# NBDsoftware/deep_cartograph

Measured on AMD Instinct MI355X. Metric: Deep-TICA training frames/sec on 10Mx512 feature matrix at 1/2/4/8 GPUs, higher is better.
Workload: dtype f32

## Files before the change

deep_cartograph_amd/csrc/gemm.h:

```cpp
#pragma once
#include <type_traits>
#include "common.h"
#include "handoff.h"

namespace dcv {

#ifdef DCV_STAMP
__device__ unsigned long long g_stamp[8 * 8192];
#define DCV_STAMP_AT(slot)                                                                      \
    do {                                                                                        \
        if (threadIdx.x == 0 && blockIdx.x < 8192 && blockIdx.z == 0)                           \
            g_stamp[blockIdx.x * 8 + (slot)] = __builtin_amdgcn_s_memtime();                   \
    } while (0)
#define DCV_STAMP_RT(slot)                                                                      \
    do {                                                                                        \
        if (threadIdx.x == 0 && blockIdx.x < 8192 && blockIdx.z == 0)                           \
            g_stamp[blockIdx.x * 8 + (slot)] = __builtin_amdgcn_s_memrealtime();               \
    } while (0)
#else
#define DCV_STAMP_AT(slot) do {} while (0)
#define DCV_STAMP_RT(slot) do {} while (0)
#endif

typedef float f32x16 __attribute__((ext_vector_type(16)));
typedef float v4f __attribute__((ext_vector_type(4)));
typedef unsigned u32x4 __attribute__((ext_vector_type(4)));
typedef __bf16 bf16x8 __attribute__((ext_vector_type(8)));

__device__ __forceinline__ void split3(const float (&x)[8], u32x4& p1, u32x4& p2, u32x4& p3) {
#pragma unroll
    for (int i = 0; i < 4; ++i) {
        const unsigned a = __float_as_uint(x[2 * i]), b = __float_as_uint(x[2 * i + 1]);
        p1[i] = __builtin_amdgcn_perm(b, a, 0x07060302);
        const float ra = x[2 * i] - __uint_as_float(a & 0xFFFF0000u);
        const float rb = x[2 * i + 1] - __uint_as_float(b & 0xFFFF0000u);
        const unsigned a2 = __float_as_uint(ra), b2 = __float_as_uint(rb);
        p2[i] = __builtin_amdgcn_perm(b2, a2, 0x07060302);
        const float sa = ra - __uint_as_float(a2 & 0xFFFF0000u);
        const float sb = rb - __uint_as_float(b2 & 0xFFFF0000u);
        p3[i] = __builtin_amdgcn_perm(__float_as_uint(sb), __float_as_uint(sa), 0x07060302);
    }
}
__device__ __forceinline__ bf16x8 as_bf16x8(const u32x4& v) { return __builtin_bit_cast(bf16x8, v); }

enum GemmMode { kNT = 0, kNN = 1, kTN = 2 };

template <class E, class = void> struct epi_has_asum : std::false_type {};
template <class E> struct epi_has_asum<E, std::void_t<decltype(E::kASum)>> : std::bool_constant<E::kASum> {};

struct RowMap {
    const int64_t* idx;
    int64_t row0;
    int32_t half;
    int32_t lag;
    template <bool GATHER>
    __device__ __forceinline__ int64_t get(int64_t r) const {
        const bool second = half > 0 && r >= half;
        const int64_t j = second ? r - half : r;
        int64_t base;
        if constexpr (GATHER) base = idx ? idx[j] : row0 + j;
        else base = row0 + j;
        return second ? base + lag : base;
    }
};
inline RowMap identity_rows() { return RowMap{nullptr, 0, 0, 0}; }

struct Operand {
    const float* p;
    int64_t ld;
    RowMap rows;
    const float* shift;
    int vec_ok;
    int planes = 0;
    int64_t pstride = 0;
};

struct GemmDims {
    int64_t M, N, K;
    int64_t k_chunk;
    int tiles_m, tiles_n;
    int xcd_remap;
    int wt;
    int tail_split = 0;
    float* tail_ws = nullptr;
    unsigned* tail_cnt = nullptr;
};

template <int WAVES_M_, int WAVES_N_, int FM_, int FN_, int KB_, int NBUF_ = 2, bool SPLIT_ = false, int PL_ = 0>
struct TileCfg {
    static constexpr int WAVES_M = WAVES_M_, WAVES_N = WAVES_N_, FM = FM_, FN = FN_, KB = KB_, NBUF = NBUF_;
    static constexpr bool SPLIT = SPLIT_;
    static constexpr int PL = PL_;
    static_assert(PL == 0 || SPLIT, "plane operands belong to the split flavour");
    static constexpr bool LS = (PL_ & 16) != 0;
    static constexpr int RAW_SZ = LS ? (WAVES_M_ * FM_ * 32 + WAVES_N_ * FN_ * 32) * KB_ : 0;
    static constexpr int A_SZ = (PL & 5) ? 3 * (WAVES_M_ * FM_ * 32) * (KB_ / 2) : (WAVES_M_ * FM_ * 32) * KB_;
    static constexpr int B_SZ = (PL & 10) ? 3 * (WAVES_N_ * FN_ * 32) * (KB_ / 2) : (WAVES_N_ * FN_ * 32) * KB_;
    static_assert(NBUF >= 2 && NBUF <= 8, "NBUF");
    static constexpr int TM = WAVES_M * FM * 32;
    static constexpr int TN = WAVES_N * FN * 32;
    static_assert(WAVES_M * WAVES_N == 4, "4 waves per workgroup");
    static_assert(KB == 16 || KB == 32, "KB");
};

template <int KB>
__device__ __forceinline__ int mmajor_off(int row, int chunk) {
    constexpr int CPR = KB / 4;
    constexpr int RPBR = 64 / KB;
    return row * KB + ((chunk ^ ((row / RPBR) % CPR)) << 2);
}

__device__ __forceinline__ void glds16(const float* gsrc, unsigned lds_wave_addr) {
    unsigned keep;
    asm volatile(
        "s_mov_b32 %0, m0\n\t"
        "s_mov_b32 m0, %2\n\t"
        "s_nop 0\n\t"
        "global_load_lds_dwordx4 %1, off\n\t"
        "s_mov_b32 m0, %0"
        : "=&s"(keep)
        : "v"(gsrc), "s"(lds_wave_addr)
        : "memory");
}
__device__ __forceinline__ unsigned lds_addr_uniform(const float* p) {
    const unsigned a = (unsigned)(uintptr_t)(__attribute__((address_space(3))) const float*)p;
    return __builtin_amdgcn_readfirstlane(a);
}

template <int PER>
__device__ __forceinline__ void glds16_batch(const float* base, const unsigned (&voff)[PER], unsigned lds0) {
    static_assert(PER == 1 || PER == 2 || PER == 4, "units per thread");
    unsigned keep;
    if constexpr (PER == 1) {
        asm volatile(
            "s_mov_b32 %0, m0\n\ts_nop 3\n\t"
            "s_mov_b32 m0, %3\n\ts_nop 0\n\tglobal_load_lds_dwordx4 %1, %2\n\t"
            "s_mov_b32 m0, %0"
            : "=&s"(keep)
            : "v"(voff[0]), "s"(base), "s"(lds0)
            : "memory");
    } else if constexpr (PER == 2) {
        asm volatile(
            "s_mov_b32 %0, m0\n\ts_nop 3\n\t"
            "s_mov_b32 m0, %4\n\ts_nop 0\n\tglobal_load_lds_dwordx4 %1, %3\n\t"
            "s_mov_b32 m0, %5\n\ts_nop 0\n\tglobal_load_lds_dwordx4 %2, %3\n\t"
            "s_mov_b32 m0, %0"
            : "=&s"(keep)
            : "v"(voff[0]), "v"(voff[1]), "s"(base), "s"(lds0), "s"(lds0 + 4096u)
            : "memory");
    } else {
        asm volatile(
            "s_mov_b32 %0, m0\n\ts_nop 3\n\t"
            "s_mov_b32 m0, %6\n\ts_nop 0\n\tglobal_load_lds_dwordx4 %1, %5\n\t"
            "s_mov_b32 m0, %7\n\ts_nop 0\n\tglobal_load_lds_dwordx4 %2, %5\n\t"
            "s_mov_b32 m0, %8\n\ts_nop 0\n\tglobal_load_lds_dwordx4 %3, %5\n\t"
            "s_mov_b32 m0, %9\n\ts_nop 0\n\tglobal_load_lds_dwordx4 %4, %5\n\t"
            "s_mov_b32 m0, %0"
            : "=&s"(keep)
            : "v"(voff[0]), "v"(voff[1]), "v"(voff[2]), "v"(voff[3]), "s"(base), "s"(lds0), "s"(lds0 + 4096u),
              "s"(lds0 + 8192u), "s"(lds0 + 12288u)
            : "memory");
    }
}
constexpr int64_t kMaxAffineLd = (int64_t)1 << 22;

template <int T, int KB, bool VEC, bool GATHER>
struct MMajorStage {
    static constexpr int CPR = KB / 4;
    static constexpr int RPBR = 64 / KB;
    static constexpr int UNITS = T * CPR;
    static constexpr int PER = (UNITS + 255) / 256;
    static_assert(256 % CPR == 0 && ((256 / CPR) / RPBR) % CPR == 0, "swizzle must not depend on the unit index");
    float4 r[PER];
    const float* src[PER];
    unsigned voff[PER];
// ... 431 lines not shown
    };
    float sha[FM], shb[FN];
    bool dma_sub = false;
#pragma unroll
    for (int i = 0; i < FM; ++i) sha[i] = 0.f;
#pragma unroll
    for (int j = 0; j < FN; ++j) shb[j] = 0.f;
    if constexpr (!A_MM) {
        if (A.shift) {
            dma_sub = true;
#pragma unroll
            for (int i = 0; i < FM; ++i) {
                const int64_t c = m0 + wm + i * 32 + (lane & 31);
                sha[i] = c < d.M ? A.shift[c] : 0.f;
            }
        }
    }
    if constexpr (!B_MM) {
        if (B.shift) {
            dma_sub = true;
#pragma unroll
            for (int j = 0; j < FN; ++j) {
                const int64_t c = n0 + wn + j * 32 + (lane & 31);
                shb[j] = c < d.N ? B.shift[c] : 0.f;
            }
        }
    }
    auto read_frags = [&](Frags& f, const float* la, const float* lb, int g) {
#pragma unroll
        for (int i = 0; i < FM; ++i) {
            if constexpr (A_MM) {
                f.a[i] = frag_mmajor<KB>(la, wm + i * 32, g, lane);
            } else {
#pragma unroll
                for (int s = 0; s < 4; ++s) f.a[i][s] = frag_kmajor<TM>(la, wm + i * 32, g, s, lane);
            }
        }
#pragma unroll
        for (int b = 0; b < NB; ++b)
#pragma unroll
            for (int j = 0; j < FN; ++j) {
                if constexpr (B_MM) {
                    f.b[b][j] = frag_mmajor<KB>(lb, wn + j * 32, g, lane);
                } else {
#pragma unroll
                    for (int s = 0; s < 4; ++s) f.b[b][j][s] = frag_kmajor<TN>(lb + b * B_SZ, wn + j * 32, g, s, lane);
                }
            }
    };
    auto sub_frags = [&](Frags& f) {
        if constexpr (!A_MM) {
#pragma unroll
            for (int i = 0; i < FM; ++i)
#pragma unroll
                for (int s = 0; s < 4; ++s) f.a[i][s] -= sha[i];
        }
        if constexpr (!B_MM) {
#pragma unroll
            for (int b = 0; b < NB; ++b)
#pragma unroll
                for (int j = 0; j < FN; ++j)
#pragma unroll
                    for (int s = 0; s < 4; ++s) f.b[b][j][s] -= shb[j];
        }
    };
    auto pin_frags = [&](Frags& f) {
        if constexpr (A_MM) {
#pragma unroll
            for (int i = 0; i < FM; ++i) asm volatile("" : "+v"(f.a[i]));
        }
        if constexpr (B_MM) {
#pragma unroll
            for (int b = 0; b < NB; ++b)
#pragma unroll
                for (int j = 0; j < FN; ++j) asm volatile("" : "+v"(f.b[b][j]));
        }
    };
    struct Frags8 {
        float a[FM][8];
        float b[NB][FN][8];
        u32x4 ap[3][FM];
        u32x4 bp[3][FN];
    };
    auto read_frags8 = [&](Frags8& f, const float* la, const float* lb, int s) {
        const int h = lane >> 5;
#pragma unroll
        for (int i = 0; i < FM; ++i) {
            if constexpr (PA) {
#pragma unroll
                for (int q = 0; q < 3; ++q)
                    f.ap[q][i] = __builtin_bit_cast(u32x4, frag_mmajor_chunk<KF>(la + q * TM * KF, wm + i * 32, 2 * s + h, lane));
            } else if constexpr (A_MM) {
                const v4f u = frag_mmajor_chunk<KB>(la, wm + i * 32, 4 * s + 2 * h, lane);
                const v4f v = frag_mmajor_chunk<KB>(la, wm + i * 32, 4 * s + 2 * h + 1, lane);
                f.a[i][0] = u.x; f.a[i][1] = u.y; f.a[i][2] = u.z; f.a[i][3] = u.w;
                f.a[i][4] = v.x; f.a[i][5] = v.y; f.a[i][6] = v.z; f.a[i][7] = v.w;
            } else {
#pragma unroll
                for (int e = 0; e < 8; ++e) f.a[i][e] = la[(16 * s + 8 * h + e) * TM + wm + i * 32 + (lane & 31)];
            }
        }
#pragma unroll
        for (int b = 0; b < NB; ++b)
#pragma unroll
            for (int j = 0; j < FN; ++j) {
                if constexpr (PB) {
#pragma unroll
                    for (int q = 0; q < 3; ++q)
                        f.bp[q][j] = __builtin_bit_cast(u32x4, frag_mmajor_chunk<KF>(lb + q * TN * KF, wn + j * 32, 2 * s + h, lane));
                } else if constexpr (B_MM) {
                    const v4f u = frag_mmajor_chunk<KB>(lb, wn + j * 32, 4 * s + 2 * h, lane);
                    const v4f v = frag_mmajor_chunk<KB>(lb, wn + j * 32, 4 * s + 2 * h + 1, lane);
                    f.b[b][j][0] = u.x; f.b[b][j][1] = u.y; f.b[b][j][2] = u.z; f.b[b][j][3] = u.w;
                    f.b[b][j][4] = v.x; f.b[b][j][5] = v.y; f.b[b][j][6] = v.z; f.b[b][j][7] = v.w;
                } else {
#pragma unroll
                    for (int e = 0; e < 8; ++e) f.b[b][j][e] = lb[b * B_SZ + (16 * s + 8 * h + e) * TN + wn + j * 32 + (lane & 31)];
                }
            }
    };
    struct Planes {
        u32x4 a1[FM], a2[FM], a3[FM], b1[NB][FN], b2[NB][FN], b3[NB][FN];
    };
    auto split_frags = [&](const Frags8& f, Planes& p) {
#pragma unroll
        for (int i = 0; i < FM; ++i) {
#ifdef DCV_ABL_NOSPLIT_A
#pragma unroll
            for (int e = 0; e < 4; ++e) {
                p.a1[i][e] = __builtin_amdgcn_perm(__float_as_uint(f.a[i][2 * e + 1]), __float_as_uint(f.a[i][2 * e]), 0x07060302);
                p.a2[i][e] = p.a1[i][e];
                p.a3[i][e] = p.a1[i][e];
            }
#else
            if constexpr (PA) {
                p.a1[i] = f.ap[0][i]; p.a2[i] = f.ap[1][i]; p.a3[i] = f.ap[2][i];
            } else {
                split3(f.a[i], p.a1[i], p.a2[i], p.a3[i]);
            }
#endif
        }
#pragma unroll
        for (int b = 0; b < NB; ++b)
#pragma unroll
            for (int j = 0; j < FN; ++j) {
                if constexpr (PB) {
                    p.b1[b][j] = f.bp[0][j]; p.b2[b][j] = f.bp[1][j]; p.b3[b][j] = f.bp[2][j];
                } else {
                    split3(f.b[b][j], p.b1[b][j], p.b2[b][j], p.b3[b][j]);
                }
            }
    };
    [[maybe_unused]] auto pin_planes = [&](Planes& p) {
#pragma unroll
        for (int i = 0; i < FM; ++i) {
            asm volatile("" : "+v"(p.a1[i]), "+v"(p.a2[i]), "+v"(p.a3[i]));
        }
#pragma unroll
        for (int b = 0; b < NB; ++b)
#pragma unroll
            for (int j = 0; j < FN; ++j) asm volatile("" : "+v"(p.b1[b][j]), "+v"(p.b2[b][j]), "+v"(p.b3[b][j]));
    };
    auto mfma_planes = [&](const Planes& p, auto&& between) {
#define DCV_SPLIT_PRODUCT(PA, PB, K)                                                                                           \
    _Pragma("unroll") for (int b = 0; b < NB; ++b) _Pragma("unroll") for (int i = 0; i < FM; ++i) _Pragma("unroll") for (int j = 0; j < FN; ++j) \
        acc[b][i][j] = __builtin_amdgcn_mfma_f32_32x32x16_bf16(as_bf16x8(p.PA[i]), as_bf16x8(p.PB[b][j]), acc[b][i][j], 0, 0, 0); \
    between(K);
        DCV_SPLIT_PRODUCT(a3, b1, 0)
        DCV_SPLIT_PRODUCT(a1, b3, 1)
        DCV_SPLIT_PRODUCT(a2, b2, 2)
        DCV_SPLIT_PRODUCT(a2, b1, 3)
        DCV_SPLIT_PRODUCT(a1, b2, 4)
        DCV_SPLIT_PRODUCT(a1, b1, 5)
#undef DCV_SPLIT_PRODUCT
    };
    auto mfma16 = [&](const Frags8& f) {
        Planes p;
        split_frags(f, p);
        mfma_planes(p, [](int) {});
    };
    constexpr bool kASum = epi_has_asum<Epi>::value && MODE == kTN && !Cfg::SPLIT;
    float asum[FM];
#pragma unroll
    for (int i = 0; i < FM; ++i) asum[i] = 0.f;
    auto add_asum = [&](const Frags& f) {
        if constexpr (kASum) {
#pragma unroll
            for (int i = 0; i < FM; ++i) asum[i] += (f.a[i][0] + f.a[i][1]) + (f.a[i][2] + f.a[i][3]);
        }
    };
    auto mfma_step = [&](const Frags& f, int s) {
#pragma unroll
        for (int b = 0; b < NB; ++b)
#pragma unroll
            for (int i = 0; i < FM; ++i)
#pragma unroll
                for (int j = 0; j < FN; ++j)
                    acc[b][i][j] = __builtin_amdgcn_mfma_f32_32x32x2f32(f.a[i][s], f.b[b][j][s], acc[b][i][j], 0, 0, 0);
    };
    auto mfma_group = [&](const Frags& f) {
#pragma unroll
        for (int s = 0; s < 4; ++s)
// ... 65 lines not shown
        float* const raw0 = lds + Cfg::NBUF * STAGE;
        const int64_t nst_ls = (k_end - k_begin) / KB;
        auto dma_raw = [&](int64_t k0, int rb) {
            float* rbuf = raw0 + rb * RAW;
            const unsigned l0 = ldsw + (unsigned)(Cfg::NBUF * STAGE + rb * RAW) * 4u;
            if (pl_a_aff) am.glds_affine(am.tile_base(A, m0_ld, k0), l0);
            else am.glds(k0, rbuf, t);
            if (pl_b_aff) bm.glds_affine(bm.tile_base(B, n0, k0), l0 + (unsigned)(TM * KB) * 4u);
            else bm.glds(k0, rbuf + TM * KB, t);
        };
        auto raw_to_regs = [&](int rb) {
            const float* rbuf = raw0 + rb * RAW;
#pragma unroll
            for (int i = 0; i < PERA; ++i) am.r[i] = *reinterpret_cast<const float4*>(rbuf + (t + 256 * i) * 4);
#pragma unroll
            for (int i = 0; i < PERB; ++i) bm.r[i] = *reinterpret_cast<const float4*>(rbuf + TM * KB + (t + 256 * i) * 4);
        };
        auto split_to_planes = [&](float* pbuf) {
            am.store_planes(pbuf, t);
            bm.store_planes(pbuf + A_SZ, t);
        };
        if (nst_ls > 0) {
            dma_raw(k_begin, 0);
            if (nst_ls > 1) {
                dma_raw(k_begin + KB, 1);
                vm_wait<PERA + PERB>();
            } else {
                vm_wait<0>();
            }
            __syncthreads();
            raw_to_regs(0);
            split_to_planes(lds);
            vm_wait<0>();
            __syncthreads();
            for (int64_t st = 0; st < nst_ls; ++st) {
                const int cur = (int)(st & 1);
                if (st + 1 < nst_ls) raw_to_regs(cur ^ 1);
                __builtin_amdgcn_sched_barrier(0);
                if (st + 2 < nst_ls) dma_raw(k_begin + (st + 2) * KB, cur);
                __builtin_amdgcn_sched_barrier(0);
                if (m0 + wm < d.M) compute_stage(lds + cur * STAGE);
                if (st + 1 < nst_ls) split_to_planes(lds + (cur ^ 1) * STAGE);
                vm_wait<0>();
                __syncthreads();
            }
        }
    }
    const bool dense_ok = !LS && (PRE || (!(PSA || PSB) && nst > 0 && stage_dense(k_begin) && affine_all()));
    const int64_t nfull = dense_ok ? (k_end - k_begin) / KB : 0;
    if (nfull > 0) {
        const int64_t nst = nfull;
        constexpr int NBUF = Cfg::NBUF;
        constexpr int GL = (A_MM ? NPA * MMajorStage<TM, KA, VEC, GATHER>::PER : KMajorStage<TM, KB, VEC, GATHER>::PER) +
                           NB * (B_MM ? NPB * MMajorStage<TN, KBB, VEC, GATHER>::PER : KMajorStage<TN, KB, VEC, GATHER>::PER);
        static_assert((NBUF - 2) * GL <= 63, "vmcnt range");
        static_assert(Cfg::SPLIT || G % 2 == 0, "fragment double buffer parity");
#pragma unroll
        for (int s = 0; s < NBUF - 1; ++s)
            if (s < nst) glds_stage(k_begin + s * KB, s);
        if constexpr (kSidePre) {
            static_assert((NBUF - 2) * GL + EPASS * ENQ <= 63, "vmcnt range");
            side_ready = epi.vec && (m0 + TM <= d.M) && (n0 + TN <= d.N);
            if constexpr (Epi::kMaskIn) side_ready = side_ready && epi.mask == nullptr;
            if (side_ready) {
                const int ec4 = t % EC4, er0 = t / EC4;
#pragma unroll
                for (int q = 0; q < EPASS * ENQ; ++q)
                    side_pre[q] = *reinterpret_cast<const float4*>(epi.side_ptr(m0 + er0 + q * ERPP, n0 + ec4 * 4));
                vm_wait_younger<NBUF - 2, GL, EPASS * ENQ>(nst - 1);
            } else {
                vm_wait_younger<NBUF - 2, GL>(nst - 1);
            }
        } else {
            vm_wait_younger<NBUF - 2, GL>(nst - 1);
        }
        __syncthreads();
#ifndef DCV_ABL_NOLOAD
        if (NBUF - 1 < nst) glds_stage(k_begin + (NBUF - 1) * KB, NBUF - 1);
#endif
        DCV_STAMP_AT(1);
        DCV_STAMP_RT(5);
        if constexpr (Cfg::SPLIT) {
            constexpr int S = KB / 16;
            Frags8 f0, f1;
#ifdef DCV_PIPE_SPLIT
            Planes pl0, pl1;
#endif
            read_frags8(f0, lds, lds + A_SZ, 0);
#ifdef DCV_PIPE_SPLIT
            if constexpr (S == 2) split_frags(f0, pl0);
#endif
            int cur_buf = 0;
            for (int64_t st = 0; st < nst; ++st) {
                const float* la = lds + cur_buf * STAGE;
                const float* lb = la + A_SZ;
                const int nxt_buf = cur_buf + 1 == NBUF ? 0 : cur_buf + 1;
#ifdef DCV_PIPE_SPLIT
                if constexpr (S == 2) {
                    constexpr int NMF = 6 * NB * FM * FN;
                    constexpr int NVA = 44 * (FM + NB * FN);
                    constexpr int VPM = (NVA + NMF - 1) / NMF;
                    read_frags8(f1, la, lb, 1);
                    mfma_planes(pl0, [](int) {});
                    split_frags(f1, pl1);
                    pin_planes(pl1);
#pragma unroll
                    for (int q = 0; q < NMF; ++q) {
                        __builtin_amdgcn_sched_group_barrier(0x008, 1, 0);
                        __builtin_amdgcn_sched_group_barrier(0x002, VPM, 0);
                    }
                    __builtin_amdgcn_sched_barrier(0);
                    vm_wait_younger<NBUF - 2, GL>(nst - 2 - st);
                    __syncthreads();
                    read_frags8(f0, lds + nxt_buf * STAGE, lds + nxt_buf * STAGE + A_SZ, 0);
                    const bool more = st + NBUF < nst;
                    const int64_t k_next = k_begin + (st + NBUF) * KB;
                    __builtin_amdgcn_sched_barrier(0);
                    if (more) glds_stage(k_next, cur_buf, 3);
                    __builtin_amdgcn_sched_barrier(0);
                    mfma_planes(pl1, [](int) {});
                    split_frags(f0, pl0);
                    pin_planes(pl0);
#pragma unroll
                    for (int q = 0; q < NMF; ++q) {
                        __builtin_amdgcn_sched_group_barrier(0x008, 1, 0);
                        __builtin_amdgcn_sched_group_barrier(0x002, VPM, 0);
                    }
                    __builtin_amdgcn_sched_barrier(0);
                } else
#endif
                if constexpr (S == 2) {
                    read_frags8(f1, la, lb, 1);
                    mfma16(f0);
                    Planes pl;
                    split_frags(f1, pl);
                    vm_wait_younger<NBUF - 2, GL>(nst - 2 - st);
#ifndef DCV_ABL_NOBARRIER
                    __syncthreads();
#endif
                    read_frags8(f0, lds + nxt_buf * STAGE, lds + nxt_buf * STAGE + A_SZ, 0);
                    const bool more = st + NBUF < nst;
                    const int64_t k_next = k_begin + (st + NBUF) * KB;
                    mfma_planes(pl, [&](int k) {
#ifndef DCV_ABL_NOLOAD
                        if (k == 0 || k == 2) {
                            __builtin_amdgcn_sched_barrier(0);
                            if (more) glds_stage(k_next, cur_buf, k == 0 ? 1 : 2);
                            __builtin_amdgcn_sched_barrier(0);
                        }
#endif
                    });
                } else {
                    vm_wait_younger<NBUF - 2, GL>(nst - 2 - st);
#ifndef DCV_ABL_NOBARRIER
                    __syncthreads();
#endif
#ifndef DCV_ABL_NOLOAD
                    if (st + NBUF < nst) glds_stage(k_begin + (st + NBUF) * KB, cur_buf);
#endif
                    read_frags8(f1, lds + nxt_buf * STAGE, lds + nxt_buf * STAGE + A_SZ, 0);
                    mfma16(f0);
                    f0 = f1;
                }
                cur_buf = nxt_buf;
            }
            __syncthreads();
        } else {
        Frags f0, f1;
        read_frags(f0, lds, lds + A_SZ, 0);
        int cur_buf = 0;
        for (int64_t st = 0; st < nst; ++st) {
            const float* la = lds + cur_buf * STAGE;
            const float* lb = la + A_SZ;
            const int nxt_buf = cur_buf + 1 == NBUF ? 0 : cur_buf + 1;
#pragma unroll
            for (int g = 0; g < G; g += 2) {
                read_frags(f1, la, lb, g + 1);
                __builtin_amdgcn_sched_barrier(0);
                pin_frags(f0);
                if (dma_sub) sub_frags(f0);
                add_asum(f0);
                mfma_group(f0);
                __builtin_amdgcn_sched_barrier(0);
                if (g + 2 < G) {
                    read_frags(f0, la, lb, g + 2);
                    __builtin_amdgcn_sched_barrier(0);
                    pin_frags(f1);
                    if (dma_sub) sub_frags(f1);
                    add_asum(f1);
                    mfma_group(f1);
                    __builtin_amdgcn_sched_barrier(0);
                } else {
                    vm_wait_younger<NBUF - 2, GL>(nst - 2 - st);
#ifndef DCV_ABL_NOBARRIER
                    __syncthreads();
#endif
                    __builtin_amdgcn_sched_barrier(0);
                    pin_frags(f1);
                    if (dma_sub) sub_frags(f1);
                    add_asum(f1);
                    mfma_step(f1, 0);
                    __builtin_amdgcn_sched_barrier(0);
#ifndef DCV_ABL_NOLOAD
                    if (st + NBUF < nst) glds_stage(k_begin + (st + NBUF) * KB, cur_buf, 1);
#endif
                    __builtin_amdgcn_sched_barrier(0);
                    mfma_step(f1, 1);
                    __builtin_amdgcn_sched_barrier(0);
#ifndef DCV_ABL_NOLOAD
                    if (st + NBUF < nst) glds_stage(k_begin + (st + NBUF) * KB, cur_buf, 2);
#endif
                    __builtin_amdgcn_sched_barrier(0);
                    mfma_step(f1, 2);
                    __builtin_amdgcn_sched_barrier(0);
                    read_frags(f0, lds + nxt_buf * STAGE, lds + nxt_buf * STAGE + A_SZ, 0);
                    __builtin_amdgcn_sched_barrier(0);
                    mfma_step(f1, 3);
                    __builtin_amdgcn_sched_barrier(0);
                }
            }
            cur_buf = nxt_buf;
        }
        __syncthreads();
        }
    } else {
        DCV_STAMP_AT(1);
        DCV_STAMP_RT(5);
    }
    const int64_t k_rem = k_begin + nfull * KB;
    const int64_t nrem = (PRE || LS) ? 0 : (k_end - k_rem + KB - 1) / KB;
    if (nrem > 0) {
        resolve_stage(k_rem);
        load_stage(k_rem);
        if (nrem > 1) resolve_stage(k_rem + KB);
        store_stage(lds);
        __syncthreads();
        for (int64_t st = 0; st < nrem; ++st) {
            const float* cur = lds + (st & 1) * STAGE;
            float* nxt = lds + ((st + 1) & 1) * STAGE;
            const bool more = st + 1 < nrem;
            if (more) {
                load_stage(k_rem + (st + 1) * KB);
                if (st + 2 < nrem) resolve_stage(k_rem + (st + 2) * KB);
            }
            if (MODE == kTN || m0 + wm < d.M) compute_stage(cur);
            if (more) store_stage(nxt);
            __syncthreads();
// ... 201 lines not shown
```

deep_cartograph_amd/csrc/gemm_kernels.h:

```cpp
#pragma once
#include <type_traits>
#include <stdlib.h>
#include <hip/hip_ext.h>
#include "gemm.h"

namespace dcv {

constexpr float kSoftplus0 = 0.6931471824645996f;
__device__ __forceinline__ float act_fwd(int act, float z) {
    switch (act) {
        case DCV_ACT_LEAKY_RELU: return z > 0.f ? z : 0.01f * z;
        case DCV_ACT_RELU: return z > 0.f ? z : 0.f;
        case DCV_ACT_TANH: return tanhf(z);
        case DCV_ACT_ELU: return z > 0.f ? z : expm1f(z);
        case DCV_ACT_SOFTPLUS: return z > 20.f ? z : log1pf(expf(z));
        case DCV_ACT_SHIFTED_SOFTPLUS: return (z > 20.f ? z : log1pf(expf(z))) - kSoftplus0;
        case DCV_ACT_CUSTOM_SIGMOID: return 1.f / (1.f + expf(-3.f * z));
        default: return z;
    }
}
__device__ __forceinline__ float act_grad_from_out(int act, float h) {
    switch (act) {
        case DCV_ACT_LEAKY_RELU: return h > 0.f ? 1.f : 0.01f;
        case DCV_ACT_RELU: return h > 0.f ? 1.f : 0.f;
// ... 409 lines not shown
        if (ws) (void)hipFree(ws);
        if (cnt) (void)hipFree(cnt);
        return false;
    }
    tw->ws = static_cast<float*>(ws);
    tw->cnt = static_cast<unsigned*>(cnt);
    tw->cap = cap;
    tw->max_tiles_n = max_tiles_n;
    return true;
}
#ifndef DCV_TAIL_STAGES_MIN
#define DCV_TAIL_STAGES_MIN 8
#endif
#ifndef DCV_TAIL_MINSTAGES
#define DCV_TAIL_MINSTAGES 2
#endif
inline int xcd_remap_enabled() {
    static const int env = [] { const char* e = getenv("DCV_XCD_REMAP"); return e ? atoi(e) : 1; }();
    return env;
}
inline bool tail_split_enabled() {
    static const bool on = [] { const char* e = getenv("DCV_TAIL_KSPLIT"); return !(e && e[0] == '0'); }();
    return on;
}

struct GemmPlan {
    GemmDims d;
    int64_t splits;
    bool vec, gather;
};
template <int MODE, class Cfg, int NB, class Epi>
static int prepare_gemm(const Operand& A, const Operand& B, int64_t M, int64_t N, int64_t K, int64_t k_chunk, const Epi& epi,
                        int* tiles_m_out, const TailWs* tw, GemmPlan* plan) {
    GemmDims& d = plan->d;
    d = GemmDims{};
    d.M = M;
    d.N = N;
    d.K = K;
    d.k_chunk = k_chunk > 0 ? k_chunk : K;
    d.tiles_m = (int)cdiv(M, Cfg::TM);
    d.tiles_n = (int)cdiv(N, Cfg::TN);
    if (tiles_m_out) *tiles_m_out = d.tiles_m;
    {
        const int env = xcd_remap_enabled();
        const int64_t nsplit = (MODE == kTN) ? cdiv(K, d.k_chunk) : 1;
        static const int wt_env = [] { const char* e = getenv("DCV_WT"); return e ? atoi(e) : 1; }();
        const int64_t out_bytes = nsplit * M * N * (int64_t)sizeof(float) * NB;
        d.wt = (wt_env != 0 && out_bytes <= (256ll << 20)) ? 1 : 0;
        d.xcd_remap = env && ((MODE == kTN) ? (nsplit % 8 == 0) : (d.tiles_m % 8 == 0 && d.tiles_n > 1));
        if constexpr (MODE != kTN && NB == 1) {
            const int64_t stages = K / Cfg::KB, ncu = num_cus();
            const int64_t all = (int64_t)d.tiles_m * d.tiles_n, regular = all - d.tiles_n;
            if (tw && tw->ws && tail_split_enabled() && M % Cfg::TM != 0 && d.tiles_m >= 2 && K % Cfg::KB == 0 && stages >= DCV_TAIL_STAGES_MIN &&
                all <= 4 * ncu && cdiv(all, ncu) > cdiv(regular, ncu) && d.tiles_n <= tw->max_tiles_n) {
                const int64_t want = stages / DCV_TAIL_MINSTAGES < kTailMaxSplit ? stages / DCV_TAIL_MINSTAGES : kTailMaxSplit;
                const int64_t kc = cdiv(stages, want) * Cfg::KB;
                const int64_t S = cdiv(K, kc);
                if (S >= 2 && (int64_t)d.tiles_n * S * Cfg::FM * Cfg::FN * 16 * 256 <= tw->cap) {
                    d.tail_split = (int)S;
                    d.k_chunk = kc;
                    d.tail_ws = tw->ws;
                    d.tail_cnt = tw->cnt;
                    d.xcd_remap = env && ((d.tiles_m - 1) % 8 == 0 && d.tiles_n > 1);
                }
            }
        }
    }
    plan->splits = (MODE == kTN) ? cdiv(K, d.k_chunk) : 1;
    const int64_t tiles = (int64_t)d.tiles_m * d.tiles_n;
    DCV_REQUIRE(tiles > 0 && tiles < (1ll << 31) && plan->splits > 0 && plan->splits < 65536, "gemm: grid out of range (tiles=%lld splits=%lld)",
                (long long)tiles, (long long)plan->splits);
    DCV_REQUIRE(!(Cfg::SPLIT && (A.shift || B.shift)), "gemm: a column shift needs the FP32-input MFMA flavour");
    if constexpr (std::is_base_of<EpiSlab, Epi>::value) {
        if (plan->splits > epi.cap) {
            set_error("gemm: %lld split-K slabs needed, the slab buffer holds %lld", (long long)plan->splits, (long long)epi.cap);
            return DCV_ENOMEM;
        }
    }
    constexpr bool A_MM = (MODE == kNT || MODE == kNN), B_MM = (MODE == kNT);
    plan->vec = A.vec_ok && B.vec_ok && (!A_MM || K % 4 == 0) && (!B_MM || K % 4 == 0);
    plan->gather = A.rows.idx != nullptr || B.rows.idx != nullptr;
    return DCV_OK;
}
template <int MODE, class Cfg, int NB, class Epi>
static int launch_gemm_cfg(const Operand& A, const Operand& B, int64_t lag2, int64_t M, int64_t N, int64_t K,
                           int64_t k_chunk, const Epi& epi, hipStream_t s, int* tiles_m_out = nullptr, const TailWs* tw = nullptr) {
    GemmPlan pl;
    const int rc = prepare_gemm<MODE, Cfg, NB, Epi>(A, B, M, N, K, k_chunk, epi, tiles_m_out, tw, &pl);
    if (rc) return rc;
    if (pl.vec && !pl.gather) return launch_gemm_vec<MODE, Cfg, NB, true, false, Epi>(A, B, lag2, pl.d, pl.splits, epi, s);
    if (pl.vec) return launch_gemm_vec<MODE, Cfg, NB, true, true, Epi>(A, B, lag2, pl.d, pl.splits, epi, s);
    return launch_gemm_vec<MODE, Cfg, NB, false, true, Epi>(A, B, lag2, pl.d, pl.splits, epi, s);
}

enum CfgPick { kPickNarrowN, kPickNarrowM, kPickHalfM, kPickQuarter, kPickBig };
template <int MODE, bool HEAD>
static CfgPick pick_cfg(int64_t M, int64_t N, int64_t K, int64_t k_chunk) {
#ifdef DCV_FORCE_BIG
    return kPickBig;
#endif
    if (N <= 32) return kPickNarrowN;
    if (M <= 32) return kPickNarrowM;
    if constexpr (MODE != kTN) {
        const int64_t want = 2 * (int64_t)num_cus();
        const int64_t tn = cdiv(N, 128);
        if (cdiv(M, 128) * tn < want) {
            if (cdiv(M, 64) * tn >= want || M <= 64 * 4) return kPickHalfM;
            if (cdiv(M, 64) * tn < want / 2) return kPickNarrowM;
            if constexpr (!HEAD) {
                static const bool quarter_off = [] { const char* e = getenv("DCV_NO_QUARTER_NT"); return e && e[0] == '1'; }();
                if (!quarter_off && N % 64 == 0) return kPickQuarter;
            }
            return kPickHalfM;
        }
    }
    if constexpr (MODE == kTN) {
        const int64_t nsplit = cdiv(K, k_chunk > 0 ? k_chunk : K);
        if (cdiv(M, 128) * cdiv(N, 128) * nsplit <= (int64_t)num_cus() / 2) return kPickQuarter;
    }
    return kPickBig;
}
template <class Cfg, class Epi>
static int launch_gemm_ls(const Operand& A, const Operand& B, int64_t M, int64_t N, int64_t K, const Epi& epi, hipStream_t s,
                          int* tiles_m_out, const TailWs* tw) {
    if (K % Cfg::KB != 0 || A.shift || B.shift) return 1;
    GemmPlan pl;
    int rc = prepare_gemm<kNT, Cfg, 1, Epi>(A, B, M, N, K, 0, epi, tiles_m_out, tw, &pl);
    if (rc) return rc;
    if (!pl.vec || pl.gather) return 1;
    return launch_gemm_vec<kNT, Cfg, 1, true, false, Epi>(A, B, 0, pl.d, pl.splits, epi, s);
}

template <int MODE, bool S, class Epi>
static int launch_gemm_mode(const Operand& A, const Operand& B, int64_t M, int64_t N, int64_t K, int64_t k_chunk,
                            const Epi& epi, hipStream_t s, int* tiles_m_out, const TailWs* tw = nullptr) {
#ifdef DCV_BIGCFG
    using Big = CfgBig;
#else
    using Big = CfgBigT<S>;
#endif
    const CfgPick pick = pick_cfg<MODE, Epi::kHead>(M, N, K, k_chunk);
#ifdef DCV_PS_EXPERIMENT
    if constexpr (S && MODE != kTN) {
        constexpr int PS = MODE == kNT ? 12 : 4;
        static const bool ps_on = [] { const char* e = getenv("DCV_SPLIT_AT_STORE"); return !(e && e[0] == '0'); }();
        if (ps_on && K % 32 == 0) {
            if (pick == kPickHalfM || (pick == kPickQuarter && Epi::kHead))
                return launch_gemm_cfg<MODE, TileCfg<2, 2, 1, 2, 32, 2, true, PS>, 1, Epi>(A, B, 0, M, N, K, k_chunk, epi, s, tiles_m_out, tw);
            if (pick == kPickNarrowM) return launch_gemm_cfg<MODE, TileCfg<1, 4, 1, 1, 32, 2, true, PS>, 1, Epi>(A, B, 0, M, N, K, k_chunk, epi, s, tiles_m_out, tw);
            if constexpr (!Epi::kHead) {
                if (pick == kPickQuarter) return launch_gemm_cfg<MODE, TileCfg<2, 2, 1, 1, 32, 2, true, PS>, 1, Epi>(A, B, 0, M, N, K, k_chunk, epi, s, tiles_m_out, tw);
            }
        }
    }
#endif
#ifdef DCV_PS_EXPERIMENT
    if constexpr (S && MODE == kNT && !Epi::kHead) {
        static const bool ls_on = [] { const char* e = getenv("DCV_LS"); return e && e[0] == '1'; }();
        if (ls_on && pick == kPickQuarter) {
            const int rc = launch_gemm_ls<TileCfg<2, 2, 1, 1, 32, 2, true, 28>, Epi>(A, B, M, N, K, epi, s, tiles_m_out, tw);
            if (rc != 1) return rc;
        }
    }
#endif
    switch (pick) {
        case kPickNarrowN: return launch_gemm_cfg<MODE, CfgNarrowNT<S>, 1, Epi>(A, B, 0, M, N, K, k_chunk, epi, s, tiles_m_out, tw);
        case kPickNarrowM: return launch_gemm_cfg<MODE, CfgNarrowMT<S>, 1, Epi>(A, B, 0, M, N, K, k_chunk, epi, s, tiles_m_out, tw);
        case kPickHalfM: return launch_gemm_cfg<MODE, CfgHalfMT<S>, 1, Epi>(A, B, 0, M, N, K, k_chunk, epi, s, tiles_m_out, tw);
        case kPickQuarter:
            if constexpr (!Epi::kHead) return launch_gemm_cfg<MODE, CfgQuarterT<S>, 1, Epi>(A, B, 0, M, N, K, k_chunk, epi, s, tiles_m_out, tw);
            else return launch_gemm_cfg<MODE, CfgHalfMT<S>, 1, Epi>(A, B, 0, M, N, K, k_chunk, epi, s, tiles_m_out, tw);
        default: return launch_gemm_cfg<MODE, Big, 1, Epi>(A, B, 0, M, N, K, k_chunk, epi, s, tiles_m_out, tw);
// ... 221 lines not shown
```

Measured before the change: 79.45 million.

## Unroll split-GEMM K loop by ring slot and precompute LDS fragment offsets

```diff
diff --git a/deep_cartograph_amd/csrc/gemm.h b/deep_cartograph_amd/csrc/gemm.h
--- a/deep_cartograph_amd/csrc/gemm.h
+++ b/deep_cartograph_amd/csrc/gemm.h
@@ -1,5 +1,6 @@
 #pragma once
 #include <type_traits>
+#include <utility>
 #include "common.h"
 #include "handoff.h"
 
@@ -45,6 +46,11 @@
 
 enum GemmMode { kNT = 0, kNN = 1, kTN = 2 };
 
+template <class F, int... Is>
+__device__ __forceinline__ void for_each_const(std::integer_sequence<int, Is...>, F&& f) {
+    (f(std::integral_constant<int, Is>{}), ...);
+}
+
 template <class E, class = void> struct epi_has_asum : std::false_type {};
 template <class E> struct epi_has_asum<E, std::void_t<decltype(E::kASum)>> : std::bool_constant<E::kASum> {};
 
@@ -86,11 +92,13 @@
     unsigned* tail_cnt = nullptr;
 };
 
-template <int WAVES_M_, int WAVES_N_, int FM_, int FN_, int KB_, int NBUF_ = 2, bool SPLIT_ = false, int PL_ = 0>
+template <int WAVES_M_, int WAVES_N_, int FM_, int FN_, int KB_, int NBUF_ = 2, bool SPLIT_ = false, int PL_ = 0, bool PIPE_ = false>
 struct TileCfg {
     static constexpr int WAVES_M = WAVES_M_, WAVES_N = WAVES_N_, FM = FM_, FN = FN_, KB = KB_, NBUF = NBUF_;
     static constexpr bool SPLIT = SPLIT_;
     static constexpr int PL = PL_;
+    static constexpr bool PIPE = PIPE_;
+    static_assert(!PIPE || (SPLIT && KB_ == 32), "the pipelined ring loop: split flavour, two 16-deep steps per stage");
     static_assert(PL == 0 || SPLIT, "plane operands belong to the split flavour");
     static constexpr bool LS = (PL_ & 16) != 0;
     static constexpr int RAW_SZ = LS ? (WAVES_M_ * FM_ * 32 + WAVES_N_ * FN_ * 32) * KB_ : 0;
@@ -688,22 +696,45 @@
         u32x4 ap[3][FM];
         u32x4 bp[3][FN];
     };
-    auto read_frags8 = [&](Frags8& f, const float* la, const float* lb, int s) {
-        const int h = lane >> 5;
+    constexpr int S16 = KB / 16;
+    constexpr int NOA = PA ? S16 : (A_MM ? 2 * S16 : 1), NOB = PB ? S16 : (B_MM ? 2 * S16 : 1);
+    static_assert((32 / (64 / KB)) % (KB / 4) == 0 && (32 / (64 / KF)) % (KF / 4) == 0, "the swizzle of a row repeats every 32 rows");
+    struct FragOff8 {
+        int a[NOA], b[NOB];
+    };
+    auto frag8_offsets = [&](FragOff8& o) {
+        const int h = lane >> 5, r = lane & 31;
+#pragma unroll
+        for (int s = 0; s < S16; ++s) {
+            if constexpr (PA) o.a[s] = mmajor_off<KF>(wm + r, 2 * s + h);
+            else if constexpr (A_MM) {
+                o.a[2 * s] = mmajor_off<KB>(wm + r, 4 * s + 2 * h);
+                o.a[2 * s + 1] = mmajor_off<KB>(wm + r, 4 * s + 2 * h + 1);
+            }
+            if constexpr (PB) o.b[s] = mmajor_off<KF>(wn + r, 2 * s + h);
+            else if constexpr (B_MM) {
+                o.b[2 * s] = mmajor_off<KB>(wn + r, 4 * s + 2 * h);
+                o.b[2 * s + 1] = mmajor_off<KB>(wn + r, 4 * s + 2 * h + 1);
+            }
+        }
+        if constexpr (!A_MM) o.a[0] = 8 * h * TM + wm + r;
+        if constexpr (!B_MM) o.b[0] = 8 * h * TN + wn + r;
+    };
+    auto read_frags8_at = [&](Frags8& f, const float* la, const float* lb, int s, const FragOff8& o) {
 #pragma unroll
         for (int i = 0; i < FM; ++i) {
             if constexpr (PA) {
 #pragma unroll
                 for (int q = 0; q < 3; ++q)
-                    f.ap[q][i] = __builtin_bit_cast(u32x4, frag_mmajor_chunk<KF>(la + q * TM * KF, wm + i * 32, 2 * s + h, lane));
+                    f.ap[q][i] = __builtin_bit_cast(u32x4, *reinterpret_cast<const v4f*>(la + q * TM * KF + i * 32 * KF + o.a[s]));
             } else if constexpr (A_MM) {
-                const v4f u = frag_mmajor_chunk<KB>(la, wm + i * 32, 4 * s + 2 * h, lane);
-                const v4f v = frag_mmajor_chunk<KB>(la, wm + i * 32, 4 * s + 2 * h + 1, lane);
+                const v4f u = *reinterpret_cast<const v4f*>(la + i * 32 * KB + o.a[2 * s]);
+                const v4f v = *reinterpret_cast<const v4f*>(la + i * 32 * KB + o.a[2 * s + 1]);
                 f.a[i][0] = u.x; f.a[i][1] = u.y; f.a[i][2] = u.z; f.a[i][3] = u.w;
                 f.a[i][4] = v.x; f.a[i][5] = v.y; f.a[i][6] = v.z; f.a[i][7] = v.w;
             } else {
 #pragma unroll
-                for (int e = 0; e < 8; ++e) f.a[i][e] = la[(16 * s + 8 * h + e) * TM + wm + i * 32 + (lane & 31)];
+                for (int e = 0; e < 8; ++e) f.a[i][e] = la[(16 * s + e) * TM + i * 32 + o.a[0]];
             }
         }
 #pragma unroll
@@ -713,17 +744,22 @@
                 if constexpr (PB) {
 #pragma unroll
                     for (int q = 0; q < 3; ++q)
-                        f.bp[q][j] = __builtin_bit_cast(u32x4, frag_mmajor_chunk<KF>(lb + q * TN * KF, wn + j * 32, 2 * s + h, lane));
+                        f.bp[q][j] = __builtin_bit_cast(u32x4, *reinterpret_cast<const v4f*>(lb + q * TN * KF + j * 32 * KF + o.b[s]));
                 } else if constexpr (B_MM) {
-                    const v4f u = frag_mmajor_chunk<KB>(lb, wn + j * 32, 4 * s + 2 * h, lane);
-                    const v4f v = frag_mmajor_chunk<KB>(lb, wn + j * 32, 4 * s + 2 * h + 1, lane);
+                    const v4f u = *reinterpret_cast<const v4f*>(lb + j * 32 * KB + o.b[2 * s]);
+                    const v4f v = *reinterpret_cast<const v4f*>(lb + j * 32 * KB + o.b[2 * s + 1]);
                     f.b[b][j][0] = u.x; f.b[b][j][1] = u.y; f.b[b][j][2] = u.z; f.b[b][j][3] = u.w;
                     f.b[b][j][4] = v.x; f.b[b][j][5] = v.y; f.b[b][j][6] = v.z; f.b[b][j][7] = v.w;
                 } else {
 #pragma unroll
-                    for (int e = 0; e < 8; ++e) f.b[b][j][e] = lb[b * B_SZ + (16 * s + 8 * h + e) * TN + wn + j * 32 + (lane & 31)];
-                }
-            }
+                    for (int e = 0; e < 8; ++e) f.b[b][j][e] = lb[b * B_SZ + (16 * s + e) * TN + j * 32 + o.b[0]];
+                }
+            }
+    };
+    auto read_frags8 = [&](Frags8& f, const float* la, const float* lb, int s) {
+        FragOff8 o;
+        frag8_offsets(o);
+        read_frags8_at(f, la, lb, s, o);
     };
     struct Planes {
         u32x4 a1[FM], a2[FM], a3[FM], b1[NB][FN], b2[NB][FN], b3[NB][FN];
@@ -955,25 +991,28 @@
         DCV_STAMP_RT(5);
         if constexpr (Cfg::SPLIT) {
             constexpr int S = KB / 16;
+            const int nsts = __builtin_amdgcn_readfirstlane((int)nst);
+            FragOff8 fo;
+            frag8_offsets(fo);
+#pragma unroll
+            for (int q = 0; q < NOA; ++q) asm volatile("" : "+v"(fo.a[q]));
+#pragma unroll
+            for (int q = 0; q < NOB; ++q) asm volatile("" : "+v"(fo.b[q]));
             Frags8 f0, f1;
-#ifdef DCV_PIPE_SPLIT
-            Planes pl0, pl1;
-#endif
-            read_frags8(f0, lds, lds + A_SZ, 0);
-#ifdef DCV_PIPE_SPLIT
-            if constexpr (S == 2) split_frags(f0, pl0);
-#endif
-            int cur_buf = 0;
-            for (int64_t st = 0; st < nst; ++st) {
-                const float* la = lds + cur_buf * STAGE;
+            [[maybe_unused]] Planes pl0, pl1;
+            read_frags8_at(f0, lds, lds + A_SZ, 0, fo);
+            if constexpr (Cfg::PIPE) split_frags(f0, pl0);
+            auto ring_stage = [&](auto slot, int st) {
+                constexpr int CUR = decltype(slot)::value, NXT = CUR + 1 == NBUF ? 0 : CUR + 1;
+                const float* la = lds + CUR * STAGE;
                 const float* lb = la + A_SZ;
-                const int nxt_buf = cur_buf + 1 == NBUF ? 0 : cur_buf + 1;
-#ifdef DCV_PIPE_SPLIT
-                if constexpr (S == 2) {
+                const float* na = lds + NXT * STAGE;
+                const float* nb = na + A_SZ;
+                if constexpr (Cfg::PIPE) {
                     constexpr int NMF = 6 * NB * FM * FN;
                     constexpr int NVA = 44 * (FM + NB * FN);
                     constexpr int VPM = (NVA + NMF - 1) / NMF;
-                    read_frags8(f1, la, lb, 1);
+                    read_frags8_at(f1, la, lb, 1, fo);
                     mfma_planes(pl0, [](int) {});
                     split_frags(f1, pl1);
                     pin_planes(pl1);
@@ -983,13 +1022,13 @@
                         __builtin_amdgcn_sched_group_barrier(0x002, VPM, 0);
                     }
                     __builtin_amdgcn_sched_barrier(0);
-                    vm_wait_younger<NBUF - 2, GL>(nst - 2 - st);
+                    vm_wait_younger<NBUF - 2, GL>(nsts - 2 - st);
                     __syncthreads();
-                    read_frags8(f0, lds + nxt_buf * STAGE, lds + nxt_buf * STAGE + A_SZ, 0);
-                    const bool more = st + NBUF < nst;
-                    const int64_t k_next = k_begin + (st + NBUF) * KB;
+                    read_frags8_at(f0, na, nb, 0, fo);
+                    const bool more = st + NBUF < nsts;
+                    const int64_t k_next = k_begin + (int64_t)(st + NBUF) * KB;
                     __builtin_amdgcn_sched_barrier(0);
-                    if (more) glds_stage(k_next, cur_buf, 3);
+                    if (more) glds_stage(k_next, CUR, 3);
                     __builtin_amdgcn_sched_barrier(0);
                     mfma_planes(pl1, [](int) {});
                     split_frags(f0, pl0);
@@ -1000,42 +1039,45 @@
                         __builtin_amdgcn_sched_group_barrier(0x002, VPM, 0);
                     }
                     __builtin_amdgcn_sched_barrier(0);
-                } else
-#endif
-                if constexpr (S == 2) {
-                    read_frags8(f1, la, lb, 1);
+                } else if constexpr (S == 2) {
+                    read_frags8_at(f1, la, lb, 1, fo);
                     mfma16(f0);
                     Planes pl;
                     split_frags(f1, pl);
-                    vm_wait_younger<NBUF - 2, GL>(nst - 2 - st);
+                    vm_wait_younger<NBUF - 2, GL>(nsts - 2 - st);
 #ifndef DCV_ABL_NOBARRIER
                     __syncthreads();
 #endif
-                    read_frags8(f0, lds + nxt_buf * STAGE, lds + nxt_buf * STAGE + A_SZ, 0);
-                    const bool more = st + NBUF < nst;
-                    const int64_t k_next = k_begin + (st + NBUF) * KB;
+                    read_frags8_at(f0, na, nb, 0, fo);
+                    const bool more = st + NBUF < nsts;
+                    const int64_t k_next = k_begin + (int64_t)(st + NBUF) * KB;
                     mfma_planes(pl, [&](int k) {
 #ifndef DCV_ABL_NOLOAD
                         if (k == 0 || k == 2) {
                             __builtin_amdgcn_sched_barrier(0);
-                            if (more) glds_stage(k_next, cur_buf, k == 0 ? 1 : 2);
+                            if (more) glds_stage(k_next, CUR, k == 0 ? 1 : 2);
                             __builtin_amdgcn_sched_barrier(0);
                         }
 #endif
                     });
                 } else {
-                    vm_wait_younger<NBUF - 2, GL>(nst - 2 - st);
+                    vm_wait_younger<NBUF - 2, GL>(nsts - 2 - st);
 #ifndef DCV_ABL_NOBARRIER
                     __syncthreads();
 #endif
 #ifndef DCV_ABL_NOLOAD
-                    if (st + NBUF < nst) glds_stage(k_begin + (st + NBUF) * KB, cur_buf);
-#endif
-                    read_frags8(f1, lds + nxt_buf * STAGE, lds + nxt_buf * STAGE + A_SZ, 0);
+                    if (st + NBUF < nsts) glds_stage(k_begin + (int64_t)(st + NBUF) * KB, CUR);
+#endif
+                    read_frags8_at(f1, na, nb, 0, fo);
                     mfma16(f0);
                     f0 = f1;
                 }
-                cur_buf = nxt_buf;
+            };
+            for (int st = 0; st < nsts; st += NBUF) {
+                for_each_const(std::make_integer_sequence<int, NBUF>{}, [&](auto slot) {
+                    constexpr int B = decltype(slot)::value;
+                    if (B == 0 || st + B < nsts) ring_stage(slot, st + B);
+                });
             }
             __syncthreads();
         } else {
diff --git a/deep_cartograph_amd/csrc/gemm_kernels.h b/deep_cartograph_amd/csrc/gemm_kernels.h
--- a/deep_cartograph_amd/csrc/gemm_kernels.h
+++ b/deep_cartograph_amd/csrc/gemm_kernels.h
@@ -515,12 +515,36 @@
     plan->gather = A.rows.idx != nullptr || B.rows.idx != nullptr;
     return DCV_OK;
 }
+template <class Cfg>
+using PipeOf = TileCfg<Cfg::WAVES_M, Cfg::WAVES_N, Cfg::FM, Cfg::FN, Cfg::KB, Cfg::NBUF, Cfg::SPLIT, Cfg::PL, true>;
+template <class Cfg, int NB>
+constexpr bool pipe_family() {
+    return Cfg::SPLIT && !Cfg::PIPE && Cfg::KB == 32 && Cfg::PL == 0 && NB == 1 && Cfg::FM == 1 && Cfg::FN == 1;
+}
+inline int pipe_mode() {
+    static const int env = [] { const char* e = getenv("DCV_PIPE"); return e ? atoi(e) : 0; }();
+    return env;
+}
+inline bool use_pipe(const GemmPlan& pl) {
+    const int mode = pipe_mode();
+    if (mode == 2) return true;
+    if (mode != 1) return false;
+    const GemmDims& d = pl.d;
+    const int64_t regular = (int64_t)(d.tail_split > 0 ? d.tiles_m - 1 : d.tiles_m) * d.tiles_n * pl.splits;
+    return regular <= (int64_t)num_cus();
+}
 template <int MODE, class Cfg, int NB, class Epi>
 static int launch_gemm_cfg(const Operand& A, const Operand& B, int64_t lag2, int64_t M, int64_t N, int64_t K,
                            int64_t k_chunk, const Epi& epi, hipStream_t s, int* tiles_m_out = nullptr, const TailWs* tw = nullptr) {
     GemmPlan pl;
     const int rc = prepare_gemm<MODE, Cfg, NB, Epi>(A, B, M, N, K, k_chunk, epi, tiles_m_out, tw, &pl);
     if (rc) return rc;
+    if constexpr (pipe_family<Cfg, NB>()) {
+        if (pl.vec && use_pipe(pl)) {
+            if (!pl.gather) return launch_gemm_vec<MODE, PipeOf<Cfg>, NB, true, false, Epi>(A, B, lag2, pl.d, pl.splits, epi, s);
+            return launch_gemm_vec<MODE, PipeOf<Cfg>, NB, true, true, Epi>(A, B, lag2, pl.d, pl.splits, epi, s);
+        }
+    }
     if (pl.vec && !pl.gather) return launch_gemm_vec<MODE, Cfg, NB, true, false, Epi>(A, B, lag2, pl.d, pl.splits, epi, s);
     if (pl.vec) return launch_gemm_vec<MODE, Cfg, NB, true, true, Epi>(A, B, lag2, pl.d, pl.splits, epi, s);
     return launch_gemm_vec<MODE, Cfg, NB, false, true, Epi>(A, B, lag2, pl.d, pl.splits, epi, s);
```

New measurement: 79.51 million, median of 2. About the same (+0.1%).
